# vice87/gam-ngs

Hardware: AMD Instinct MI355X
Metric: GCUPS (higher is better)
Workload: dtype int32 (fast blocks: exact packed-f16 offsets from per-lane int32 bases, two tasks per register; results bit-identical to the reference's int64 DP)

## Files before the change

### gam_ngs_amd/csrc/kernel_pair.inc

```
#ifndef GAMDP_PACKED_TOP
#define GAMDP_PACKED_TOP 1
#endif
typedef _Float16 h2 __attribute__((ext_vector_type(2)));
__device__ __forceinline__ h2 as_h2(u32 x) { return __builtin_bit_cast(h2, x); }
__device__ __forceinline__ u32 as_u(h2 x) { return __builtin_bit_cast(u32, x); }
constexpr u32 PK_NINF = 0xFC00FC00u;
constexpr u32 PK_PINF = 0x7C007C00u;

__device__ __forceinline__ u32 pk(const _Float16 lo, const _Float16 hi) { const h2 v = {lo, hi}; return as_u(v); }
__device__ __forceinline__ _Float16 lo_of(const u32 v) { return as_h2(v).x; }
__device__ __forceinline__ _Float16 hi_of(const u32 v) { return as_h2(v).y; }

__device__ __forceinline__ _Float16 g4_to_h(const int g4, const int base)
{
    if (g4 <= NEG / 2) return lo_of(PK_NINF);
    return (_Float16)(float)((g4 >> 2) - base);
}
__device__ __forceinline__ int h_to_g4(const _Float16 h, const int base)
{
    const float f = (float)h;
    if (!(f > -60000.0f)) return NEG;
    if (!(f < 60000.0f)) return 0;
    return 4 * ((int)f + base);
}

template <int C, int LPT>
struct PairFmt {
    typedef Strip<LPT, true> ST;
    static constexpr bool GRP = (LPT == QL);
    static constexpr u32 CK_LANE = GRP ? 24u : (u32)LANE_WORDS<C>;
    static_assert(!GRP || C + 4 <= 24, "checkpoint row of the eight-task kernel");
    static constexpr u32 CK_ROWS = 64u * CK_LANE;
    static constexpr u32 CK_WORDS = GRP ? CK_ROWS : CK_ROWS + 128;
    static constexpr u32 BND_VALS = ST::BND_WORDS;
    static constexpr u32 BND_WORDS = GRP ? ST::BND_WORDS : ST::BND_WORDS + 2u * ST::NB;
    static constexpr int RC = 4;
};
__shared__ u32 s_ringB2[RING_B + ROWS];
__shared__ u32 s_pcap[QT][2][20];

__device__ __forceinline__ u32 pk_sel(const u32 codeA, const u32 codeB) { return 0x000C000Cu | (codeA << 8) | ((4u + codeB) << 24); }
__device__ __forceinline__ u32 pk_tab(const u32 codeb) { return 0x44444444u + (0x03u << (codeb * 8u)); }

__device__ __forceinline__ u32 code2_at(gcptr p2, int64_t idx) { return (p2[idx >> 4] >> ((idx & 15) * 2)) & 3u; }

__shared__ u32 s_oB2[QT][64 + ROWS];
template <int C, int LPT>
struct PRing {
    typedef typename std::conditional<LPT == 64, const u32*, const uint16_t*>::type APtr;
    static constexpr int SZ = QRing<C>::SZ;
    static __device__ __forceinline__ void put_a(const int sub, const int k, const u32 codeA, const u32 codeB)
    {
        if constexpr (LPT == 64) RingA<C>::put(k, pk_sel(codeA, codeB));
        else {
            const u32 pos = (u32)k % (u32)SZ;
            const uint16_t v = (uint16_t)(codeA | ((4u + codeB) << 8));
            s_oA16[sub][pos] = v;
            if (pos < ROWS) s_oA16[sub][pos + SZ] = v;
        }
    }
    static __device__ __forceinline__ void put_b(const int sub, const int k, const u32 ta, const u32 tb)
    {
        if constexpr (LPT == 64) {
            const int pb = k & (RING_B - 1);
            s_ringB[pb] = ta; s_ringB2[pb] = tb;
            if (pb < ROWS) { s_ringB[pb + RING_B] = ta; s_ringB2[pb + RING_B] = tb; }
        } else {
            const int pb = k & 63;
            s_qB[sub][pb] = ta; s_oB2[sub][pb] = tb;
            if (pb < ROWS) { s_qB[sub][pb + 64] = ta; s_oB2[sub][pb + 64] = tb; }
        }
    }
    static __device__ __forceinline__ APtr a_lane(const int tau0, const int lane)
    {
        if constexpr (LPT == 64) return s_ringA + (u32)((tau0 + (C - 1) * (lane + 1)) >> 4) % (u32)RingA<C>::COLS;
        else return s_oA16[lane >> 4] + (u32)(tau0 + (C - 1) * ((lane & (QL - 1)) + 1)) % (u32)SZ;
    }
    static __device__ __forceinline__ u32 a_read(APtr p, const int r)
    {
        if constexpr (LPT == 64) return p[r * RingA<C>::COLS];
        else return __builtin_amdgcn_perm(0x0C0C0C0Cu, (u32)p[r], 0x01040004u);
    }
    static __device__ __forceinline__ const u32* b_lane(const int tau0, const int lane, const int half)
    {
        if constexpr (LPT == 64) return (half ? s_ringB2 : s_ringB) + ((tau0 - lane) & (RING_B - 1));
        else return (half ? s_oB2[lane >> 4] : s_qB[lane >> 4]) + ((tau0 - (lane & (QL - 1))) & 63);
    }
    template <int C2>
    static __device__ __forceinline__ _Float16 cap_pick(const int wlane, const int half, const u32 (&Lp)[C2], const int idx)
    {
        const int lane = wlane & (LPT - 1);
        if constexpr (LPT == 64) {
            u32* const cb = (u32*)s_cap[half][lane & 1];
#pragma unroll
            for (int c = 0; c < C2; ++c) cb[c] = Lp[c];
            const u32 v = cb[idx];
            return half ? hi_of(v) : lo_of(v);
        } else {
            u32* const cb = s_pcap[wlane >> 4][lane & 1];
#pragma unroll
            for (int c = 0; c < C2; ++c) cb[c] = Lp[c];
            return __builtin_bit_cast(_Float16, reinterpret_cast<const uint16_t*>(cb)[2 * idx + half]);
        }
    }
    static constexpr u32 MARK_A = 13u, MARK_B = 9u;
    template <bool MARK = false>
    static __device__ __forceinline__ void produce(const int T, const int lane, const u32 awA, const u32 awB, const u32 bwA, const u32 bwB, const int km1A = 0, const int km1B = 0)
    {
        const int r = lane & (QL - 1);
        if (LPT == QL || lane < ROWS) {
            const int k = T + (C - 1) * LPT + r;
            u32 cA = (awA >> (2 * r)) & 3u, cB = (awB >> (2 * r)) & 3u;
            if constexpr (MARK) { cA = (k == km1A) ? MARK_A : cA; cB = (k == km1B) ? MARK_B : cB; }
            put_a(lane >> 4, k, cA, cB);
            put_b(lane >> 4, T + r, pk_tab((bwA >> (2 * r)) & 3u), pk_tab((bwB >> (2 * r)) & 3u));
        }
    }
    template <bool MARK = false>
    static __device__ __forceinline__ void prime(const Tk& ta, const Tk& tb, const int blk, const int lane, const int km1A = 0, const int km1B = 0)
    {
        const int T0 = blk * ROWS, tl = lane & (LPT - 1), sub = lane >> 4;
        const int64_t A0a = ta.a_base + ta.begin_a - ta.band, A0b = tb.a_base + tb.begin_a - tb.band;
        for (int k = T0 + tl; k < T0 + ROWS + (C - 1) * LPT; k += LPT) {
            u32 cA = code2_at(ta.a2, A0a + k), cB = code2_at(tb.a2, A0b + k);
            if constexpr (MARK) { cA = (k == km1A) ? MARK_A : cA; cB = (k == km1B) ? MARK_B : cB; }
            put_a(sub, k, cA, cB);
        }
        const int64_t Ba = ta.b_base + ta.begin_b, Bb = tb.b_base + tb.begin_b;
        for (int k = T0 - (LPT - 1) + tl; k <= T0 + ROWS - 1; k += LPT) put_b(sub, k, pk_tab(code2_at(ta.b2, Ba + k)), pk_tab(code2_at(tb.b2, Bb + k)));
    }
};

template <int C, bool HASN, bool UNTAGGED, int LPT>
__device__ __forceinline__ void single_prime(const Tk& t, const int blk, const int wlane, u32 (&W)[C + 15])
{
    typedef Ring<C, LPT, HASN> RG;
    const int T0 = blk * ROWS, lane = wlane & (LPT - 1), sub = wlane >> 4;
    const int64_t A0 = t.a_base + t.begin_a - t.band, BB = t.b_base + t.begin_b;
    for (int k = T0 + lane; k < T0 + ROWS + (C - 1) * LPT; k += LPT) RG::put_a(sub, k, code2_at(t.a2, A0 + k), false);
    for (int k = T0 - (LPT - 1) + lane; k <= T0 + ROWS - 1; k += LPT)
        RG::put_b(sub, k, enc_b<HASN>(code2_at(t.b2, BB + k), false) - (UNTAGGED ? RING_TAG<HASN> : 0u));
    const int64_t s0 = A0 + (int64_t)(C - 1) * lane + T0;
    const u32 ab = fetch16(t.a2, s0), ab2 = (C - 1 > 16) ? fetch16(t.a2, s0 + 16) : 0u;
#pragma unroll
    for (int k = 0; k < C - 1; ++k) W[k] = (k < 16) ? enc_a<HASN>((ab >> (2 * k)) & 3u, false) : enc_a<HASN>((ab2 >> (2 * (k - 16))) & 3u, false);
#pragma unroll
    for (int k = C - 1; k < C + 15; ++k) W[k] = 0;
}

template <int C, int LPT>
__device__ __forceinline__ void ck_store(gptr ck, const int wlane, const u32 (&Lp)[C], const int baseA, const int baseB)
{
    typedef PairFmt<C, LPT> FMT;
    if constexpr (FMT::GRP) {
        const u32 rA = (u32)lane_shl1<LPT>(baseA, baseA), rB = (u32)lane_shl1<LPT>(baseB, baseB);
        gptr row = ck + (u32)wlane * FMT::CK_LANE;
#pragma unroll
        for (int g = 0; g < 6; ++g) {
            auto w = [&](const int i) -> u32 { return i < C ? Lp[i < C ? i : 0] : (i == C ? (u32)baseA : (i == C + 1 ? (u32)baseB : (i == C + 2 ? rA : (i == C + 3 ? rB : 0u)))); };
            const u32x4 q = {w(4 * g), w(4 * g + 1), w(4 * g + 2), w(4 * g + 3)};
            *(g4ptr)(row + 4 * g) = q;
        }
    } else {
        img_store<C, true>(ck, wlane, Lp);
        ck[FMT::CK_ROWS + wlane] = (u32)baseA;
        ck[FMT::CK_ROWS + 64 + wlane] = (u32)baseB;
    }
}

template <int C, int LPT>
__device__ __forceinline__ int cap_limit(const Tk& t, const int lane) { return max(0, min(C, t.Y - C * lane)); }
template <int LPT>
__device__ __forceinline__ void cap_table(const int wlane, const int half, const int E0, const int R0, const int P0, const int L0)
{
    if ((wlane & (LPT - 1)) == 0) {
        const int4 e = {E0, R0, P0, L0};
        *reinterpret_cast<int4*>(s_captab[LPT == 64 ? 0 : wlane >> 4][half]) = e;
    }
}
template <int C, int CE, int LPT, bool LAST>
__device__ __forceinline__ void side_capture(const int wlane, const int half, const int T, const int base, const u32 (&Lp)[C], const int cap_max, giptr const cap_slot)
{
    const int lane = wlane & (LPT - 1);
    const int4 e = *reinterpret_cast<const int4*>(s_captab[LPT == 64 ? 0 : wlane >> 4][half]);
    const int cE = e.x - (C - 1) * lane - T;
    if ((u32)cE < (u32)cap_max && T <= e.y + lane) {
        const _Float16 vE = PRing<C, LPT>::cap_pick(wlane, half, Lp, cE);
        cap_slot[e.z - lane + T] = (int)(float)vE + base + 8 * (lane - e.x - T);
    }
    if constexpr (LAST) {
        if (T == e.y + lane && cap_max > 0) {
            giptr const lp = cap_slot + (e.w + C * lane);
            const int k1 = base - 16 * e.y - 8 * C * lane;
            auto put = [&](const int c) __attribute__((always_inline)) { lp[c] = (int)(float)(half ? hi_of(Lp[c]) : lo_of(Lp[c])) + (k1 - 8 * c); };
#pragma unroll
            for (int c = 0; c <= CE; ++c) put(c);
            if (cap_max == C) {
#pragma unroll
                for (int c = CE + 1; c < C; ++c) put(c);
            }
        }
    }
}

template <int C, int CE, bool END, int LPT = 64>
__device__ __noinline__ void pair_range(BlockState<C>* sta, BlockState<C>* stb, const Tk* tpa, const Tk* tpb, const int blk_begin_, const int blk_end_, const int wlane)
{
    static_assert(CE >= 0 && CE < C - 1 && (LPT == QL || (C - 1) % 16 == 0), "band 512 on 64 lanes (transposed ring A) or band 150 on 16");
    typedef PRing<C, LPT> PR;
    const Tk ta = load_tk<LPT>(tpa), tb = load_tk<LPT>(tpb);
    const int blk_begin = uni(blk_begin_), blk_end = uni(blk_end_);
    const int lane = wlane & (LPT - 1);
    const int LE = (ta.Y - 1) / C;
    u32 Lp[C], W[C + 15];
    int baseA, baseB;
    u32 Lin, dL, dR;
    {
        baseA = (sta->Lp[0] <= NEG / 2) ? 0 : (sta->Lp[0] >> 2);
        baseB = (stb->Lp[0] <= NEG / 2) ? 0 : (stb->Lp[0] >> 2);
#pragma unroll
        for (int c = 0; c < C; ++c) Lp[c] = pk(g4_to_h(sta->Lp[c], baseA), g4_to_h(stb->Lp[c], baseB));
        Lin = pk(g4_to_h(sta->Lin, baseA), g4_to_h(stb->Lin, baseB));
        const int lA = __shfl_up(baseA, 1, LPT), lB = __shfl_up(baseB, 1, LPT), rA = __shfl_down(baseA, 1, LPT), rB = __shfl_down(baseB, 1, LPT);
        const bool hasL = lane >= 1 && lane <= LE, hasR = lane < LE;
        dL = hasL ? pk((_Float16)(float)(lA - baseA), (_Float16)(float)(lB - baseB)) : 0u;
        dR = hasR ? pk((_Float16)(float)(rA - baseA), (_Float16)(float)(rB - baseB)) : 0u;
        const int T0 = blk_begin * ROWS;
        const int64_t sa = ta.a_base + ta.begin_a - ta.band + (int64_t)(C - 1) * lane + T0, sb = tb.a_base + tb.begin_a - tb.band + (int64_t)(C - 1) * lane + T0;
        const u32 wa = fetch16(ta.a2, sa), wb = fetch16(tb.a2, sb);
        const u32 wa2 = (C - 1 > 16) ? fetch16(ta.a2, sa + 16) : 0u, wb2 = (C - 1 > 16) ? fetch16(tb.a2, sb + 16) : 0u;
#pragma unroll
        for (int k = 0; k < C - 1; ++k)
            W[k] = (k < 16) ? pk_sel((wa >> (2 * k)) & 3u, (wb >> (2 * k)) & 3u) : pk_sel((wa2 >> (2 * (k - 16))) & 3u, (wb2 >> (2 * (k - 16))) & 3u);
#pragma unroll
        for (int k = C - 1; k < C + 15; ++k) W[k] = 0;
    }
    PR::prime(ta, tb, blk_begin, wlane);

    const int64_t iAa = ta.a_base + ta.begin_a - ta.band + (C - 1) * LPT, iBa = ta.b_base + ta.begin_b;
    const int64_t iAb = tb.a_base + tb.begin_a - tb.band + (C - 1) * LPT, iBb = tb.b_base + tb.begin_b;
    gcptr paA = ta.a2 + (iAa >> 4), pbA = ta.b2 + (iBa >> 4), paB = tb.a2 + (iAb >> 4), pbB = tb.b2 + (iBb >> 4);
    const u32 shaA = (u32)(iAa & 15) * 2u, shbA = (u32)(iBa & 15) * 2u, shaB = (u32)(iAb & 15) * 2u, shbB = (u32)(iBb & 15) * 2u;
    u32 aA_lo = paA[blk_begin + 1], aA_hi = paA[blk_begin + 2], bA_lo = pbA[blk_begin + 1], bA_hi = pbA[blk_begin + 2];
    u32 aB_lo = paB[blk_begin + 1], aB_hi = paB[blk_begin + 2], bB_lo = pbB[blk_begin + 1], bB_hi = pbB[blk_begin + 2];
    asm volatile("" : "+v"(aA_lo), "+v"(aA_hi), "+v"(bA_lo), "+v"(bA_hi), "+v"(aB_lo), "+v"(aB_hi), "+v"(bB_lo), "+v"(bB_hi));
    const h2 three = {(_Float16)3.0f, (_Float16)3.0f};
    const bool no_up = lane == LE;
    typedef Strip<LPT, true> ST;
    typedef PairFmt<C, LPT> FMT;
    constexpr int NB = ST::NB, FI = ST::FI;
    const int sshift = uni(ta.sshift);
    const bool edge = ST::opens_strip(wlane, sshift);
    const u32 my_slot = ST::slot_of(wlane, sshift);
    const u64 edge_mask = __ballot(edge);
    u32* const s_bnd = ST::staging();
    u32* const sb = s_bnd + my_slot;
    gptr const ckpt = ta.ckpt, bnd = ta.bnd;
    int xkeep = (int)PK_NINF;
    const int prio_R = uni(ta.prio_R), prio_nblk = uni(ta.prio_nblk);
    const int cap_max = END ? cap_limit<C, LPT>(ta, lane) : 0;
    giptr const cap_slot = (giptr)unip(ta.dir);
    if constexpr (END) {
        cap_table<LPT>(wlane, 0, ta.eaRel, ta.X - 1, (int)(ta.adh - cap_slot) - ta.iA, (int)(ta.lastrow - cap_slot));
        cap_table<LPT>(wlane, 1, tb.eaRel, tb.X - 1, (int)(tb.adh - cap_slot) - tb.iA, (int)(tb.lastrow - cap_slot));
    }
    constexpr bool ROT = (C + 15 == 32);
    auto block_body = [&](auto phase, const int blk) __attribute__((always_inline)) {
        constexpr int WO = ROT ? 16 * decltype(phase)::value : 0;
#define WX(i) (ROT ? (((i) + WO) & 31) : (i))
        const int T = (blk + 1) * ROWS, tau0 = blk * ROWS;
        if (prio_R != 0 && (blk & 7) == 0) set_prio_by_remaining(prio_nblk - blk, prio_R);
        const u32 aA_nx = paA[blk + 3], bA_nx = pbA[blk + 3], aB_nx = paB[blk + 3], bB_nx = pbB[blk + 3];
        PR::produce(T, wlane, __builtin_amdgcn_alignbit(aA_hi, aA_lo, shaA), __builtin_amdgcn_alignbit(aB_hi, aB_lo, shaB),
                    __builtin_amdgcn_alignbit(bA_hi, bA_lo, shbA), __builtin_amdgcn_alignbit(bB_hi, bB_lo, shbB));
        if ((blk & 3) == 0) ck_store<C, LPT>(ckpt + (u64)(blk >> 2) * FMT::CK_WORDS, wlane, Lp, baseA, baseB);
        if constexpr (!FMT::GRP) {
            if (edge) {
                gptr bb = bnd + (u64)blk * FMT::BND_WORDS + FMT::BND_VALS;
                bb[my_slot] = (u32)baseA;
                bb[NB + my_slot] = (u32)baseB;
            }
        }
        const typename PR::APtr ringA_lane = PR::a_lane(tau0, wlane);
        const u32* const rbA = PR::b_lane(tau0, wlane, 0);
        const u32* const rbB = PR::b_lane(tau0, wlane, 1);
        {
            u32 tA[2], tB[2];
            u32 m[3], D[2];
            u32 L = Lin, x = PK_NINF, Lrecv = Lin;
            W[WX(C - 1)] = PR::a_read(ringA_lane, 0);
            tA[0] = rbA[0]; tB[0] = rbB[0];
            W[WX(C)] = PR::a_read(ringA_lane, 1);
            tA[1] = rbA[1]; tB[1] = rbB[1];
            auto do_perm = [&](const int g) __attribute__((always_inline)) {
                const int r = g / C, c = g % C;
                m[g % 3] = __builtin_amdgcn_perm(tB[r & 1], tA[r & 1], W[WX(r + c)]);
            };
            auto do_fma = [&](const int g) __attribute__((always_inline)) {
                D[g % 2] = as_u(__builtin_elementwise_fma(as_h2(m[g % 3]), three, as_h2(Lp[g % C])));
            };
            auto do_max = [&](const int g) __attribute__((always_inline)) {
                const int c = g % C;
                h2 U = as_h2((c < C - 1) ? Lp[(c < C - 1) ? c + 1 : c] : x);
                if (c == CE) U = as_h2(no_up ? PK_NINF : as_u(U));
                L = as_u(__builtin_elementwise_maximum(__builtin_elementwise_maximum(as_h2(D[g % 2]), U), as_h2(L)));
                Lp[c] = L;
            };
            do_perm(0); do_perm(1); do_fma(0);
            __builtin_amdgcn_sched_barrier(0);
            static_for<ROWS>([&](auto rc) __attribute__((always_inline)) {
                constexpr int r = decltype(rc)::value;
#pragma unroll
                for (int c = 0; c < C; ++c) {
                    const int g = r * C + c;
                    if (c == 0) {
                        L = Lin; Lrecv = Lin;
                        do_fma(g + 1);
                        do_max(g);
                        do_perm(g + 2);
                    } else {
                        do_max(g);
                        if (g + 1 < ROWS * C) do_fma(g + 1);
                        if (g + 2 < ROWS * C) do_perm(g + 2);
                    }
                    if (c == 2) xkeep = lane_shl1<LPT>(xkeep, (int)Lp[0]);
                    if (c == 3) {
                        x = as_u(as_h2((u32)xkeep) + as_h2(dR));
                        lds_store2_masked<4 * (r % FI) * NB, 4 * (NB * FI + (r % FI) * NB)>(sb, Lrecv, Lp[0], edge_mask);
                    }
                    __builtin_amdgcn_sched_barrier(0);
                }
                if constexpr (r + 2 < ROWS) { W[WX(C + 1 + r)] = PR::a_read(ringA_lane, r + 2); tA[r & 1] = rbA[r + 2]; tB[r & 1] = rbB[r + 2]; }
                Lin = (u32)lane_shr1<LPT>((int)Lin, (int)L);
                Lin = as_u(as_h2(Lin) + as_h2(dL));
                __builtin_amdgcn_sched_barrier(0);
                if constexpr (END) {
                    side_capture<C, CE, LPT, true>(wlane, 0, tau0 + r, baseA, Lp, cap_max, cap_slot);
                    side_capture<C, CE, LPT, true>(wlane, 1, tau0 + r, baseB, Lp, cap_max, cap_slot);
                }
                if ((r % FI) == FI - 1) {
                    constexpr u32 PER = 2u * NB * FI / 64u;
                    const u32 w0 = (u32)wlane * PER;
                    const u32* src = s_bnd + ST::staging_index(w0);
                    gptr bp = bnd + (u64)blk * FMT::BND_WORDS + (u32)(r / FI) * (u32)(2 * NB * FI) + w0;
#pragma unroll
                    for (u32 k = 0; k < PER; k += 4) {
                        const u32x4 v = {src[k * NB], src[(k + 1) * NB], src[(k + 2) * NB], src[(k + 3) * NB]};
                        *(g4ptr)(bp + k) = v;
                    }
                }
            });
        }
#ifdef GAMDP_DIAG
        {
            u32 mIn = 0, mOut = 0;
#pragma unroll
            for (int c = 0; c < C; ++c) {
                const u32 a = Lp[c] & 0x7FFF7FFFu;
                if (c <= CE) mIn = as_u(__builtin_elementwise_max(as_h2(mIn), as_h2(a)));
                else mOut = as_u(__builtin_elementwise_max(as_h2(mOut), as_h2(a)));
            }
            if (lane >= 1) mIn = as_u(__builtin_elementwise_max(as_h2(mIn), as_h2(Lin & 0x7FFF7FFFu)));
            const u32 xv = as_u(as_h2((u32)xkeep) + as_h2(dR)) & 0x7FFF7FFFu;
            if (blk > blk_begin) mOut = as_u(__builtin_elementwise_max(as_h2(mOut), as_h2(xv)));
            if (lane < LE) mIn = as_u(__builtin_elementwise_max(as_h2(mIn), as_h2(mOut)));
            if (lane <= LE) {
                if (!((float)lo_of(mIn) < 2040.0f)) ta.pos0[-1] = 1;
                if (!((float)hi_of(mIn) < 2040.0f)) tb.pos0[-1] = 1;
            }
        }
#endif
        if ((blk & (FMT::RC - 1)) == FMT::RC - 1 || blk + 1 == blk_end) {
            const float fa = (float)lo_of(Lp[0]), fb = (float)hi_of(Lp[0]);
            const bool oka = fa > -60000.0f && fa < 60000.0f, okb = fb > -60000.0f && fb < 60000.0f;
            const u32 d = pk(oka ? lo_of(Lp[0]) : (_Float16)0.0f, okb ? hi_of(Lp[0]) : (_Float16)0.0f);
            baseA += oka ? (int)fa : 0;
            baseB += okb ? (int)fb : 0;
#pragma unroll
            for (int c = 0; c < C; ++c) Lp[c] = as_u(as_h2(Lp[c]) - as_h2(d));
            Lin = as_u(as_h2(Lin) - as_h2(d));
            const u32 dl = (u32)lane_shr1<LPT>((int)d, (int)d);
            const u32 dr = (u32)lane_shl1<LPT>((int)d, (int)d);
            if (lane >= 1 && lane <= LE) dL = as_u(as_h2(dL) + as_h2(dl) - as_h2(d));
            if (lane < LE) dR = as_u(as_h2(dR) + as_h2(dr) - as_h2(d));
        }
        if constexpr (!ROT) {
#pragma unroll
            for (int k = 0; k < C - 1; ++k) W[k] = W[k + ROWS];
        }
        aA_lo = aA_hi; aA_hi = aA_nx; bA_lo = bA_hi; bA_hi = bA_nx;
        aB_lo = aB_hi; aB_hi = aB_nx; bB_lo = bB_hi; bB_hi = bB_nx;
#undef WX
    };
    if constexpr (ROT) {
        int blk = blk_begin;
        for (; blk + 1 < blk_end; blk += 2) {
            block_body(std::integral_constant<int, 0>{}, blk);
            block_body(std::integral_constant<int, 1>{}, blk + 1);
        }
        if (blk < blk_end) block_body(std::integral_constant<int, 0>{}, blk);
    } else {
        for (int blk = blk_begin; blk < blk_end; ++blk) block_body(std::integral_constant<int, 0>{}, blk);
    }
#pragma unroll
    for (int c = 0; c < C; ++c) {
        sta->Lp[c] = h_to_g4(lo_of(Lp[c]), baseA); stb->Lp[c] = h_to_g4(hi_of(Lp[c]), baseB);
        sta->acc[c] = 0; stb->acc[c] = 0;
    }
    sta->Lin = h_to_g4(lo_of(Lin), baseA); stb->Lin = h_to_g4(hi_of(Lin), baseB);
    sta->Lout = sta->Lp[C - 1]; stb->Lout = stb->Lp[C - 1];
}

template <int C, int CE, int LPT = 64, bool FS = false>
__device__ __noinline__ void pair_top_range(BlockState<C>* sta, BlockState<C>* stb, const Tk* tpa, const Tk* tpb, const int blk_begin_, const int blk_end_, const int wlane)
{
    static_assert(CE >= 0 && CE < C - 1 && (LPT == QL || (C - 1) % 16 == 0), "band 512 on 64 lanes (transposed ring A) or band 150 on 16");
    typedef PRing<C, LPT> PR;
    const Tk ta = load_tk<LPT>(tpa), tb = load_tk<LPT>(tpb);
    const int blk_begin = uni(blk_begin_), blk_end = uni(blk_end_);
    const int lane = wlane & (LPT - 1);
    const int LE = (ta.Y - 1) / C;
    const int T0 = blk_begin * ROWS;
    const int km1A = ta.band - ta.begin_a - 1, km1B = tb.band - tb.begin_a - 1;
    const int zk = 8 * km1A, zkB = 8 * km1B;
    u32 Lp[C], W[C + 15];
    int baseA, baseB;
    u32 Lin, dL, dR;
    {
        const int rp = T0 - lane - 1, p0 = ta.begin_a + rp + C * lane - ta.band;
        const int p0B = tb.begin_a + rp + C * lane - tb.band;
        const bool dead0 = p0 < -1 && lane <= LE;
        const bool dead0B = p0B < -1 && lane <= LE;
        baseA = (sta->Lp[0] <= NEG / 2) ? 0 : (sta->Lp[0] >> 2);
        baseB = (stb->Lp[0] <= NEG / 2) ? 0 : (stb->Lp[0] >> 2);
        if (dead0) baseA = 16 * rp + 8 * C * lane;
        if (dead0B) baseB = 16 * rp + 8 * C * lane;
#pragma unroll
        for (int c = 0; c < C; ++c) {
            const bool dead = p0 + c < -1 && lane <= LE, deadB = p0B + c < -1 && lane <= LE;
            Lp[c] = pk(dead ? lo_of(PK_NINF) : g4_to_h(sta->Lp[c], baseA), deadB ? lo_of(PK_NINF) : g4_to_h(stb->Lp[c], baseB));
        }
        Lin = pk(dead0 ? lo_of(PK_NINF) : g4_to_h(sta->Lin, baseA), dead0B ? lo_of(PK_NINF) : g4_to_h(stb->Lin, baseB));
        const int lA = __shfl_up(baseA, 1, LPT), lB = __shfl_up(baseB, 1, LPT), rA = __shfl_down(baseA, 1, LPT), rB = __shfl_down(baseB, 1, LPT);
        const bool hasL = lane >= 1 && lane <= LE, hasR = lane < LE;
        dL = hasL ? pk((_Float16)(float)(lA - baseA), (_Float16)(float)(lB - baseB)) : 0u;
        dR = hasR ? pk((_Float16)(float)(rA - baseA), (_Float16)(float)(rB - baseB)) : 0u;
        const int64_t sa = ta.a_base + ta.begin_a - ta.band + (int64_t)(C - 1) * lane + T0, sb = tb.a_base + tb.begin_a - tb.band + (int64_t)(C - 1) * lane + T0;
        const u32 wa = fetch16(ta.a2, sa), wb = fetch16(tb.a2, sb);
        const u32 wa2 = (C - 1 > 16) ? fetch16(ta.a2, sa + 16) : 0u, wb2 = (C - 1 > 16) ? fetch16(tb.a2, sb + 16) : 0u;
        const int w0k = (C - 1) * lane + T0;
#pragma unroll
        for (int k = 0; k < C - 1; ++k) {
            const u32 cA = (k < 16) ? (wa >> (2 * k)) & 3u : (wa2 >> (2 * (k - 16))) & 3u, cB = (k < 16) ? (wb >> (2 * k)) & 3u : (wb2 >> (2 * (k - 16))) & 3u;
            W[k] = pk_sel((w0k + k == km1A) ? PR::MARK_A : cA, (w0k + k == km1B) ? PR::MARK_B : cB);
        }
#pragma unroll
        for (int k = C - 1; k < C + 15; ++k) W[k] = 0;
    }
    PR::template prime<true>(ta, tb, blk_begin, wlane, km1A, km1B);
    const int64_t iAa = ta.a_base + ta.begin_a - ta.band + (C - 1) * LPT, iBa = ta.b_base + ta.begin_b;
    const int64_t iAb = tb.a_base + tb.begin_a - tb.band + (C - 1) * LPT, iBb = tb.b_base + tb.begin_b;
    gcptr paA = ta.a2 + (iAa >> 4), pbA = ta.b2 + (iBa >> 4), paB = tb.a2 + (iAb >> 4), pbB = tb.b2 + (iBb >> 4);
    const u32 shaA = (u32)(iAa & 15) * 2u, shbA = (u32)(iBa & 15) * 2u, shaB = (u32)(iAb & 15) * 2u, shbB = (u32)(iBb & 15) * 2u;
    u32 aA_lo = paA[blk_begin + 1], aA_hi = paA[blk_begin + 2], bA_lo = pbA[blk_begin + 1], bA_hi = pbA[blk_begin + 2];
    u32 aB_lo = paB[blk_begin + 1], aB_hi = paB[blk_begin + 2], bB_lo = pbB[blk_begin + 1], bB_hi = pbB[blk_begin + 2];
    const h2 three = {(_Float16)3.0f, (_Float16)3.0f};
    const bool no_up = lane == LE;
    typedef Strip<LPT, true> ST;
    typedef PairFmt<C, LPT> FMT;
    constexpr int NB = ST::NB, FI = ST::FI;
    const int sshift = uni(ta.sshift);
    const bool edge = ST::opens_strip(wlane, sshift);
    const u32 my_slot = ST::slot_of(wlane, sshift);
    const u64 edge_mask = __ballot(edge);
    u32* const s_bnd = ST::staging();
    u32* const sb = s_bnd + my_slot;
    gptr const ckpt = ta.ckpt, bnd = ta.bnd;
    int xkeep = (int)PK_NINF;
    auto hf = [](const int v) -> _Float16 { return (_Float16)(float)v; };
    int g0A = baseA, g0B = baseB;
    const int cap_max = cap_limit<C, LPT>(ta, lane);
    giptr const cap_slot = (giptr)unip(ta.dir);
    cap_table<LPT>(wlane, 0, ta.band - ta.begin_a, ta.X - 1, (int)(ta.pos0 - cap_slot), 0);
    cap_table<LPT>(wlane, 1, tb.band - tb.begin_a, tb.X - 1, (int)(tb.pos0 - cap_slot), 0);
    for (int blk = blk_begin; blk < blk_end; ++blk) {
        const int T = (blk + 1) * ROWS, tau0 = blk * ROWS;
        const u32 aA_nx = paA[blk + 3], bA_nx = pbA[blk + 3], aB_nx = paB[blk + 3], bB_nx = pbB[blk + 3];
        PR::template produce<true>(T, wlane, __builtin_amdgcn_alignbit(aA_hi, aA_lo, shaA), __builtin_amdgcn_alignbit(aB_hi, aB_lo, shaB),
                                   __builtin_amdgcn_alignbit(bA_hi, bA_lo, shbA), __builtin_amdgcn_alignbit(bB_hi, bB_lo, shbB), km1A, km1B);
        if ((blk & 3) == 0) {
            ck_store<C, LPT>(ckpt + (u64)(blk >> 2) * FMT::CK_WORDS, wlane, Lp, baseA, baseB);
            g0A = baseA; g0B = baseB;
        }
        if constexpr (!FMT::GRP) {
            if (edge) {
                gptr bb = bnd + (u64)blk * FMT::BND_WORDS + FMT::BND_VALS;
                bb[my_slot] = (u32)baseA;
                bb[NB + my_slot] = (u32)baseB;
            }
        }
        const u32 Kpk = FMT::GRP ? pk(hf(baseA - g0A), hf(baseB - g0B)) : 0u;
        const typename PR::APtr ringA_lane = PR::a_lane(tau0, wlane);
        const u32* const rbA = PR::b_lane(tau0, wlane, 0);
        const u32* const rbB = PR::b_lane(tau0, wlane, 1);
        static_for<ROWS>([&](auto rc) __attribute__((always_inline)) {
            constexpr int r = decltype(rc)::value;
            W[C - 1 + r] = PR::a_read(ringA_lane, r);
            const u32 tabA = rbA[r], tabB = rbB[r];
            const int row = tau0 + r - lane;
            const int zg = 8 * row + zk, zgB = 8 * row + zkB;
            const bool zA = row <= km1A && lane <= LE, zB = row <= km1B && lane <= LE;
            const u32 Z = pk(zA ? hf(min(max(zg - baseA, -60000), 60000)) : lo_of(PK_NINF), zB ? hf(min(max(zgB - baseB, -60000), 60000)) : lo_of(PK_NINF));
            u32 ZL = Z;
            if constexpr (FS) {
                const bool gA = ta.fs && row > FORCE_MAXGAP, gB = tb.fs && row > FORCE_MAXGAP;
                ZL = (gA ? 0x0000FC00u : (Z & 0x0000FFFFu)) | (gB ? 0xFC000000u : (Z & 0xFFFF0000u));
            }
            const u32 Lrecv = Lin;
            u32 L = Lin, x = PK_NINF;
            auto cell = [&](const int c) __attribute__((always_inline)) {
                const u32 m = __builtin_amdgcn_perm(tabB, tabA, W[r + c]);
                const h2 D = __builtin_elementwise_fma(as_h2(m), three, as_h2(Lp[c]));
                h2 U = as_h2((c < C - 1) ? Lp[(c < C - 1) ? c + 1 : c] : x);
                if (c == CE) U = as_h2(no_up ? PK_NINF : as_u(U));
                L = as_u(__builtin_elementwise_maximum(__builtin_elementwise_maximum(D, U), as_h2(L)));
                Lp[c] = as_u(__builtin_elementwise_max(as_h2(L), as_h2(Z)));
                L = FS ? as_u(__builtin_elementwise_max(as_h2(L), as_h2(ZL))) : Lp[c];
            };
            cell(0);
            xkeep = lane_shl1<LPT>(xkeep, (int)Lp[0]);
            x = as_u(as_h2((u32)xkeep) + as_h2(dR));
            lds_store2_masked<4 * (r % FI) * NB, 4 * (NB * FI + (r % FI) * NB)>(sb, FMT::GRP ? as_u(as_h2(Lrecv) + as_h2(Kpk)) : Lrecv,
                                                                               FMT::GRP ? as_u(as_h2(Lp[0]) + as_h2(Kpk)) : Lp[0], edge_mask);
#pragma unroll
            for (int c = 1; c < C; ++c) cell(c);
            Lin = (u32)lane_shr1<LPT>((int)Lin, (int)L);
            Lin = as_u(as_h2(Lin) + as_h2(dL));
            side_capture<C, CE, LPT, false>(wlane, 0, tau0 + r, baseA, Lp, cap_max, cap_slot);
            side_capture<C, CE, LPT, false>(wlane, 1, tau0 + r, baseB, Lp, cap_max, cap_slot);
            if ((r % FI) == FI - 1) {
                constexpr u32 PER = 2u * NB * FI / 64u;
                const u32 w0 = (u32)wlane * PER;
                const u32* src = s_bnd + ST::staging_index(w0);
                gptr bp = bnd + (u64)blk * FMT::BND_WORDS + (u32)(r / FI) * (u32)(2 * NB * FI) + w0;
#pragma unroll
                for (u32 k = 0; k < PER; k += 4) {
                    const u32x4 v = {src[k * NB], src[(k + 1) * NB], src[(k + 2) * NB], src[(k + 3) * NB]};
                    *(g4ptr)(bp + k) = v;
                }
            }
        });
        {
            const float fa = (float)lo_of(Lp[0]), fb = (float)hi_of(Lp[0]);
            const int rpn = T - lane - 1;
            const bool followA = lane <= LE && ta.begin_a + rpn + C * lane - ta.band < -1, followB = lane <= LE && tb.begin_a + rpn + C * lane - tb.band < -1;
            const bool oka = !followA && fa > -60000.0f && fa < 60000.0f, okb = !followB && fb > -60000.0f && fb < 60000.0f;
            const _Float16 step = (_Float16)(float)(16 * ROWS);
            const u32 d = pk(oka ? lo_of(Lp[0]) : (followA ? step : (_Float16)0.0f), okb ? hi_of(Lp[0]) : (followB ? step : (_Float16)0.0f));
            baseA += oka ? (int)fa : (followA ? 16 * ROWS : 0);
            baseB += okb ? (int)fb : (followB ? 16 * ROWS : 0);
#pragma unroll
            for (int c = 0; c < C; ++c) Lp[c] = as_u(as_h2(Lp[c]) - as_h2(d));
            Lin = as_u(as_h2(Lin) - as_h2(d));
            const u32 dl = (u32)lane_shr1<LPT>((int)d, (int)d);
            const u32 dr = (u32)lane_shl1<LPT>((int)d, (int)d);
            if (lane >= 1 && lane <= LE) dL = as_u(as_h2(dL) + as_h2(dl) - as_h2(d));
            if (lane < LE) dR = as_u(as_h2(dR) + as_h2(dr) - as_h2(d));
        }
#pragma unroll
        for (int k = 0; k < C - 1; ++k) W[k] = W[k + ROWS];
        aA_lo = aA_hi; aA_hi = aA_nx; bA_lo = bA_hi; bA_hi = bA_nx;
        aB_lo = aB_hi; aB_hi = aB_nx; bB_lo = bB_hi; bB_hi = bB_nx;
    }
#pragma unroll
    for (int c = 0; c < C; ++c) {
        sta->Lp[c] = h_to_g4(lo_of(Lp[c]), baseA); stb->Lp[c] = h_to_g4(hi_of(Lp[c]), baseB);
        sta->acc[c] = 0; stb->acc[c] = 0;
    }
    sta->Lin = h_to_g4(lo_of(Lin), baseA); stb->Lin = h_to_g4(hi_of(Lin), baseB);
    sta->Lout = sta->Lp[C - 1]; stb->Lout = stb->Lp[C - 1];
}

template <int C, bool HASN, bool UNTAGGED, int LPT = 64>
__device__ __noinline__ void single_resume(BlockState<C>* st, const Tk* tp, const int blk_, const int lane)
{
    const Tk t = load_tk<LPT>(tp);
    u32 W[C + 15];
    single_prime<C, HASN, UNTAGGED, LPT>(t, uni(blk_), lane, W);
#pragma unroll
    for (int k = 0; k < C - 1; ++k) st->W[k] = W[k];
}
```

Baseline: 14230.

## Replace packed f16 FMA with integer add inside a fixed binade

For the 64-lane two-task kernel, DP values are re-centred around 1024 so every f16 value stays in the binade [1024, 2048). Within that range a fixed integer added to the bit pattern equals an f16 add of the score. The packed FMA with 3 is therefore replaced by a plain 32-bit integer add of precomputed substitution bit offsets from new select and table encodings. The cost is re-centring every 2 blocks instead of 4, with a static assert bounding column count, plus extra diagnostic checks of the binade invariant.

```diff
diff --git a/gam_ngs_amd/csrc/kernel_pair.inc b/gam_ngs_amd/csrc/kernel_pair.inc
--- a/gam_ngs_amd/csrc/kernel_pair.inc
+++ b/gam_ngs_amd/csrc/kernel_pair.inc
@@ -24,6 +24,8 @@
     return 4 * ((int)f + base);
 }
 
+constexpr int PK_MISMATCH = 12, PK_MATCH = 21;
+constexpr bool pk_binade_fits(const int c, const int rc, const int center) { return center + (c - 1) * PK_MATCH + rc * ROWS * PK_MATCH < 2 * center; }
 template <int C, int LPT>
 struct PairFmt {
     typedef Strip<LPT, true> ST;
@@ -34,13 +36,21 @@
     static constexpr u32 CK_WORDS = GRP ? CK_ROWS : CK_ROWS + 128;
     static constexpr u32 BND_VALS = ST::BND_WORDS;
     static constexpr u32 BND_WORDS = GRP ? ST::BND_WORDS : ST::BND_WORDS + 2u * ST::NB;
-    static constexpr int RC = 4;
+    static constexpr bool IADD = (LPT == 64);
+    static constexpr int CENTER = IADD ? 1024 : 0;
+    static constexpr int RC = IADD ? 2 : 4;
+    static_assert(!IADD || pk_binade_fits(C, RC, CENTER), "integer add: every value between two re-centrings stays inside the binade [1024, 2048)");
 };
+static_assert(pk_binade_fits(17, 2, 1024) && !pk_binade_fits(17, 4, 1024) && !pk_binade_fits(19, 2, 1024), "17 columns: every 2 blocks (2 032), not every 4; 19 columns: every block");
 __shared__ u32 s_ringB2[RING_B + ROWS];
 __shared__ u32 s_pcap[QT][2][20];
 
 __device__ __forceinline__ u32 pk_sel(const u32 codeA, const u32 codeB) { return 0x000C000Cu | (codeA << 8) | ((4u + codeB) << 24); }
 __device__ __forceinline__ u32 pk_tab(const u32 codeb) { return 0x44444444u + (0x03u << (codeb * 8u)); }
+__device__ __forceinline__ u32 pk_sel_i(const u32 codeA, const u32 codeB) { return 0x0C000C00u | codeA | ((4u + codeB) << 16); }
+__device__ __forceinline__ u32 pk_tab_i(const u32 codeb) { return 0x0C0C0C0Cu + (9u << (codeb * 8u)); }
+template <bool IADD> __device__ __forceinline__ u32 pk_sel_of(const u32 codeA, const u32 codeB) { return IADD ? pk_sel_i(codeA, codeB) : pk_sel(codeA, codeB); }
+template <bool IADD> __device__ __forceinline__ u32 pk_tab_of(const u32 codeb) { return IADD ? pk_tab_i(codeb) : pk_tab(codeb); }
 
 __device__ __forceinline__ u32 code2_at(gcptr p2, int64_t idx) { return (p2[idx >> 4] >> ((idx & 15) * 2)) & 3u; }
 
@@ -49,9 +59,11 @@
 struct PRing {
     typedef typename std::conditional<LPT == 64, const u32*, const uint16_t*>::type APtr;
     static constexpr int SZ = QRing<C>::SZ;
+    template <bool IADD = false>
     static __device__ __forceinline__ void put_a(const int sub, const int k, const u32 codeA, const u32 codeB)
     {
-        if constexpr (LPT == 64) RingA<C>::put(k, pk_sel(codeA, codeB));
+        static_assert(!IADD || LPT == 64, "the integer-add cell is the two-task kernel's");
+        if constexpr (LPT == 64) RingA<C>::put(k, pk_sel_of<IADD>(codeA, codeB));
         else {
             const u32 pos = (u32)k % (u32)SZ;
             const uint16_t v = (uint16_t)(codeA | ((4u + codeB) << 8));
@@ -104,7 +116,7 @@
         }
     }
     static constexpr u32 MARK_A = 13u, MARK_B = 9u;
-    template <bool MARK = false>
+    template <bool MARK = false, bool IADD = false>
     static __device__ __forceinline__ void produce(const int T, const int lane, const u32 awA, const u32 awB, const u32 bwA, const u32 bwB, const int km1A = 0, const int km1B = 0)
     {
         const int r = lane & (QL - 1);
@@ -112,11 +124,11 @@
             const int k = T + (C - 1) * LPT + r;
             u32 cA = (awA >> (2 * r)) & 3u, cB = (awB >> (2 * r)) & 3u;
             if constexpr (MARK) { cA = (k == km1A) ? MARK_A : cA; cB = (k == km1B) ? MARK_B : cB; }
-            put_a(lane >> 4, k, cA, cB);
-            put_b(lane >> 4, T + r, pk_tab((bwA >> (2 * r)) & 3u), pk_tab((bwB >> (2 * r)) & 3u));
-        }
-    }
-    template <bool MARK = false>
+            put_a<IADD>(lane >> 4, k, cA, cB);
+            put_b(lane >> 4, T + r, pk_tab_of<IADD>((bwA >> (2 * r)) & 3u), pk_tab_of<IADD>((bwB >> (2 * r)) & 3u));
+        }
+    }
+    template <bool MARK = false, bool IADD = false>
     static __device__ __forceinline__ void prime(const Tk& ta, const Tk& tb, const int blk, const int lane, const int km1A = 0, const int km1B = 0)
     {
         const int T0 = blk * ROWS, tl = lane & (LPT - 1), sub = lane >> 4;
@@ -124,10 +136,10 @@
         for (int k = T0 + tl; k < T0 + ROWS + (C - 1) * LPT; k += LPT) {
             u32 cA = code2_at(ta.a2, A0a + k), cB = code2_at(tb.a2, A0b + k);
             if constexpr (MARK) { cA = (k == km1A) ? MARK_A : cA; cB = (k == km1B) ? MARK_B : cB; }
-            put_a(sub, k, cA, cB);
+            put_a<IADD>(sub, k, cA, cB);
         }
         const int64_t Ba = ta.b_base + ta.begin_b, Bb = tb.b_base + tb.begin_b;
-        for (int k = T0 - (LPT - 1) + tl; k <= T0 + ROWS - 1; k += LPT) put_b(sub, k, pk_tab(code2_at(ta.b2, Ba + k)), pk_tab(code2_at(tb.b2, Bb + k)));
+        for (int k = T0 - (LPT - 1) + tl; k <= T0 + ROWS - 1; k += LPT) put_b(sub, k, pk_tab_of<IADD>(code2_at(ta.b2, Ba + k)), pk_tab_of<IADD>(code2_at(tb.b2, Bb + k)));
     }
 };
 
@@ -208,6 +220,8 @@
 {
     static_assert(CE >= 0 && CE < C - 1 && (LPT == QL || (C - 1) % 16 == 0), "band 512 on 64 lanes (transposed ring A) or band 150 on 16");
     typedef PRing<C, LPT> PR;
+    constexpr bool IADD = PairFmt<C, LPT>::IADD;
+    constexpr int CENTER = PairFmt<C, LPT>::CENTER;
     const Tk ta = load_tk<LPT>(tpa), tb = load_tk<LPT>(tpb);
     const int blk_begin = uni(blk_begin_), blk_end = uni(blk_end_);
     const int lane = wlane & (LPT - 1);
@@ -216,8 +230,8 @@
     int baseA, baseB;
     u32 Lin, dL, dR;
     {
-        baseA = (sta->Lp[0] <= NEG / 2) ? 0 : (sta->Lp[0] >> 2);
-        baseB = (stb->Lp[0] <= NEG / 2) ? 0 : (stb->Lp[0] >> 2);
+        baseA = (sta->Lp[0] <= NEG / 2) ? 0 : (sta->Lp[0] >> 2) - CENTER;
+        baseB = (stb->Lp[0] <= NEG / 2) ? 0 : (stb->Lp[0] >> 2) - CENTER;
 #pragma unroll
         for (int c = 0; c < C; ++c) Lp[c] = pk(g4_to_h(sta->Lp[c], baseA), g4_to_h(stb->Lp[c], baseB));
         Lin = pk(g4_to_h(sta->Lin, baseA), g4_to_h(stb->Lin, baseB));
@@ -231,11 +245,11 @@
         const u32 wa2 = (C - 1 > 16) ? fetch16(ta.a2, sa + 16) : 0u, wb2 = (C - 1 > 16) ? fetch16(tb.a2, sb + 16) : 0u;
 #pragma unroll
         for (int k = 0; k < C - 1; ++k)
-            W[k] = (k < 16) ? pk_sel((wa >> (2 * k)) & 3u, (wb >> (2 * k)) & 3u) : pk_sel((wa2 >> (2 * (k - 16))) & 3u, (wb2 >> (2 * (k - 16))) & 3u);
+            W[k] = (k < 16) ? pk_sel_of<IADD>((wa >> (2 * k)) & 3u, (wb >> (2 * k)) & 3u) : pk_sel_of<IADD>((wa2 >> (2 * (k - 16))) & 3u, (wb2 >> (2 * (k - 16))) & 3u);
 #pragma unroll
         for (int k = C - 1; k < C + 15; ++k) W[k] = 0;
     }
-    PR::prime(ta, tb, blk_begin, wlane);
+    PR::template prime<false, IADD>(ta, tb, blk_begin, wlane);
 
     const int64_t iAa = ta.a_base + ta.begin_a - ta.band + (C - 1) * LPT, iBa = ta.b_base + ta.begin_b;
     const int64_t iAb = tb.a_base + tb.begin_a - tb.band + (C - 1) * LPT, iBb = tb.b_base + tb.begin_b;
@@ -244,7 +258,6 @@
     u32 aA_lo = paA[blk_begin + 1], aA_hi = paA[blk_begin + 2], bA_lo = pbA[blk_begin + 1], bA_hi = pbA[blk_begin + 2];
     u32 aB_lo = paB[blk_begin + 1], aB_hi = paB[blk_begin + 2], bB_lo = pbB[blk_begin + 1], bB_hi = pbB[blk_begin + 2];
     asm volatile("" : "+v"(aA_lo), "+v"(aA_hi), "+v"(bA_lo), "+v"(bA_hi), "+v"(aB_lo), "+v"(aB_hi), "+v"(bB_lo), "+v"(bB_hi));
-    const h2 three = {(_Float16)3.0f, (_Float16)3.0f};
     const bool no_up = lane == LE;
     typedef Strip<LPT, true> ST;
     typedef PairFmt<C, LPT> FMT;
@@ -271,8 +284,8 @@
         const int T = (blk + 1) * ROWS, tau0 = blk * ROWS;
         if (prio_R != 0 && (blk & 7) == 0) set_prio_by_remaining(prio_nblk - blk, prio_R);
         const u32 aA_nx = paA[blk + 3], bA_nx = pbA[blk + 3], aB_nx = paB[blk + 3], bB_nx = pbB[blk + 3];
-        PR::produce(T, wlane, __builtin_amdgcn_alignbit(aA_hi, aA_lo, shaA), __builtin_amdgcn_alignbit(aB_hi, aB_lo, shaB),
-                    __builtin_amdgcn_alignbit(bA_hi, bA_lo, shbA), __builtin_amdgcn_alignbit(bB_hi, bB_lo, shbB));
+        PR::template produce<false, IADD>(T, wlane, __builtin_amdgcn_alignbit(aA_hi, aA_lo, shaA), __builtin_amdgcn_alignbit(aB_hi, aB_lo, shaB),
+                                          __builtin_amdgcn_alignbit(bA_hi, bA_lo, shbA), __builtin_amdgcn_alignbit(bB_hi, bB_lo, shbB));
         if ((blk & 3) == 0) ck_store<C, LPT>(ckpt + (u64)(blk >> 2) * FMT::CK_WORDS, wlane, Lp, baseA, baseB);
         if constexpr (!FMT::GRP) {
             if (edge) {
@@ -297,7 +310,11 @@
                 m[g % 3] = __builtin_amdgcn_perm(tB[r & 1], tA[r & 1], W[WX(r + c)]);
             };
             auto do_fma = [&](const int g) __attribute__((always_inline)) {
-                D[g % 2] = as_u(__builtin_elementwise_fma(as_h2(m[g % 3]), three, as_h2(Lp[g % C])));
+                if constexpr (IADD) D[g % 2] = m[g % 3] + Lp[g % C];
+                else {
+                    const h2 three = {(_Float16)3.0f, (_Float16)3.0f};
+                    D[g % 2] = as_u(__builtin_elementwise_fma(as_h2(m[g % 3]), three, as_h2(Lp[g % C])));
+                }
             };
             auto do_max = [&](const int g) __attribute__((always_inline)) {
                 const int c = g % C;
@@ -364,16 +381,36 @@
             const u32 xv = as_u(as_h2((u32)xkeep) + as_h2(dR)) & 0x7FFF7FFFu;
             if (blk > blk_begin) mOut = as_u(__builtin_elementwise_max(as_h2(mOut), as_h2(xv)));
             if (lane < LE) mIn = as_u(__builtin_elementwise_max(as_h2(mIn), as_h2(mOut)));
-            if (lane <= LE) {
-                if (!((float)lo_of(mIn) < 2040.0f)) ta.pos0[-1] = 1;
-                if (!((float)hi_of(mIn) < 2040.0f)) tb.pos0[-1] = 1;
+            if constexpr (!IADD) {
+                if (lane <= LE) {
+                    if (!((float)lo_of(mIn) < 2040.0f)) ta.pos0[-1] = 1;
+                    if (!((float)hi_of(mIn) < 2040.0f)) tb.pos0[-1] = 1;
+                }
+            } else {
+                u32 lIn = PK_PINF, lOut = PK_PINF, hIn = 0, hOut = 0;
+#pragma unroll
+                for (int c = 0; c < C; ++c) {
+                    if (c <= CE) { lIn = as_u(__builtin_elementwise_min(as_h2(lIn), as_h2(Lp[c]))); hIn = as_u(__builtin_elementwise_max(as_h2(hIn), as_h2(Lp[c]))); }
+                    else { lOut = as_u(__builtin_elementwise_min(as_h2(lOut), as_h2(Lp[c]))); hOut = as_u(__builtin_elementwise_max(as_h2(hOut), as_h2(Lp[c]))); }
+                }
+                if (lane < LE) { lIn = as_u(__builtin_elementwise_min(as_h2(lIn), as_h2(lOut))); hIn = as_u(__builtin_elementwise_max(as_h2(hIn), as_h2(hOut))); }
+                u32 mX = 0;
+                if (lane >= 1) mX = Lin & 0x7FFF7FFFu;
+                if (blk > blk_begin && lane < LE) mX = as_u(__builtin_elementwise_max(as_h2(mX), as_h2(xv)));
+                if (lane <= LE) {
+                    const float lo = (float)CENTER, hi = (float)(2 * CENTER);
+                    if (!((float)lo_of(lIn) >= lo && (float)lo_of(hIn) < hi && (float)lo_of(mX) < hi)) ta.pos0[-1] = 1;
+                    if (!((float)hi_of(lIn) >= lo && (float)hi_of(hIn) < hi && (float)hi_of(mX) < hi)) tb.pos0[-1] = 1;
+                }
             }
         }
 #endif
         if ((blk & (FMT::RC - 1)) == FMT::RC - 1 || blk + 1 == blk_end) {
-            const float fa = (float)lo_of(Lp[0]), fb = (float)hi_of(Lp[0]);
-            const bool oka = fa > -60000.0f && fa < 60000.0f, okb = fb > -60000.0f && fb < 60000.0f;
-            const u32 d = pk(oka ? lo_of(Lp[0]) : (_Float16)0.0f, okb ? hi_of(Lp[0]) : (_Float16)0.0f);
+            const bool inband = !IADD || lane <= LE;
+            const float fa = IADD ? (float)lo_of(Lp[0]) - (float)CENTER : (float)lo_of(Lp[0]), fb = IADD ? (float)hi_of(Lp[0]) - (float)CENTER : (float)hi_of(Lp[0]);
+            const bool oka = inband && fa > -60000.0f && fa < 60000.0f, okb = inband && fb > -60000.0f && fb < 60000.0f;
+            const _Float16 da = IADD ? (_Float16)fa : lo_of(Lp[0]), db = IADD ? (_Float16)fb : hi_of(Lp[0]);
+            const u32 d = pk(oka ? da : (_Float16)0.0f, okb ? db : (_Float16)0.0f);
             baseA += oka ? (int)fa : 0;
             baseB += okb ? (int)fb : 0;
 #pragma unroll
```

Result: no change. 14320, median of 6 (+0.7%).
